# saforem2/l2hmc

Measured on AMD Instinct MI355X. Metric: leapfrog-steps/sec (whole node), 8x8 U(1) batch 2048, 10 LF, higher is better.
Workload: dtype f32; 1 GPU; U(1) 8x8 lattice, beta=2.0, batch 2048 per GPU, 10 LF steps, GenericNet H=512 (BASELINE.json configs[2]); global_batch=2048, num_steps=10, parallelism=chains sharded over 1 GPU(s) (weak scaling), weights replicated

## Files before the change

include/l2hmc_hip.h:

```cpp
#ifndef L2HMC_HIP_H
#define L2HMC_HIP_H

#include <stddef.h>
#include <stdint.h>

#ifdef __cplusplus
extern "C" {
#endif

#define L2HMC_OK 0
#define L2HMC_ERR_ARG 1
#define L2HMC_ERR_HIP 2
#define L2HMC_ERR_WORKSPACE 3

#define L2HMC_ABI_VERSION 1

typedef void* l2hmc_stream_t;

int l2hmc_abi_version(void);
const char* l2hmc_last_error(void);

int l2hmc_u1_action_force(const float* x, int64_t rows, int32_t T, int32_t X, float beta,
                          float* action, float* force, float* avg_plaq, float* top_charge,
                          l2hmc_stream_t stream);
// ... 37 lines not shown
size_t l2hmc_stq_ws_bytes(int64_t rows, int32_t H);

int l2hmc_stq_dense(const l2hmc_dense_net* net, const float* a, const float* b, const float* bmask,
                    float t_cos, float t_sin, int64_t rows, float* S, float* T, float* Q,
                    void* ws, size_t ws_bytes, l2hmc_stream_t stream);

size_t l2hmc_stq_conv3d_ws_bytes(int64_t rows, int32_t H, int32_t T, int32_t X, int32_t F);
int l2hmc_stq_conv3d(const l2hmc_conv3d_front* front, const l2hmc_dense_net* net, int32_t T, int32_t X,
                     const float* a, const float* b, const float* bmask, float t_cos, float t_sin,
                     int64_t rows, float* S, float* Tr, float* Q, void* ws, size_t ws_bytes,
                     l2hmc_stream_t stream);

int l2hmc_lf_update_v(const float* v, const float* grad, const float* S, const float* T,
                      const float* Q, float eps, int32_t dir, int64_t rows, int32_t D,
                      float* v_out, float* logdet, l2hmc_stream_t stream);
int l2hmc_lf_update_x(const float* x, const float* v, const float* keep, const float* S,
                      const float* T, const float* Q, float eps, int32_t dir, int64_t rows,
                      int32_t D, float* x_out, float* logdet, l2hmc_stream_t stream);

int l2hmc_accept_prob(const float* h_old, const float* h_new, const float* sumlogdet, int64_t n,
                      float* p, l2hmc_stream_t stream);

int l2hmc_mix_accept(const float* x, const float* xf, const float* vf, const float* pf,
                     const float* xb, const float* vb, const float* pb, const float* coin,
                     const float* u, int32_t strict, int64_t B, int32_t D, float* x_prop,
                     float* v_prop, float* p, float* x_out, l2hmc_stream_t stream);

#define L2HMC_PLAN_LAYERED 1
#define L2HMC_PLAN_CONV3D 2
#define L2HMC_PLAN_SELECTED_ONLY 4
#define L2HMC_PLAN_RECOMPUTE 8
#define L2HMC_PLAN_TILES16_ONLY 16
#define L2HMC_PLAN_ALL_COLUMNS 32
typedef struct l2hmc_gauge_plan {
  int32_t T, X;
  int32_t num_steps;
  int32_t hmc;
  float eps;
  int32_t flags;
  const float* masks;
  l2hmc_dense_net xnet;
  l2hmc_dense_net vnet;
  l2hmc_conv3d_front xfront;
  l2hmc_conv3d_front vfront;
  const void* heads;
} l2hmc_gauge_plan;

size_t l2hmc_gauge_pack_heads_bytes(const l2hmc_gauge_plan* plan);
int l2hmc_gauge_pack_heads(const l2hmc_gauge_plan* plan, void* heads, l2hmc_stream_t stream);

size_t l2hmc_gauge_ws_bytes(const l2hmc_gauge_plan* plan, int64_t rows);

int l2hmc_gauge_plan_fused(const l2hmc_gauge_plan* plan);

int l2hmc_gauge_step_plan(int64_t rows_all, int32_t cus, int64_t* rows_out, int32_t* rows_per_wg_out);

int l2hmc_gauge_leapfrog(const l2hmc_gauge_plan* plan, float beta, int32_t step, float* x, float* v,
                         const int32_t* dir, int64_t rows, float* logdet, void* ws, size_t ws_bytes,
                         l2hmc_stream_t stream);

int l2hmc_gauge_trajectory(const l2hmc_gauge_plan* plan, float beta, const float* x0, const float* v0,
                           const int32_t* dir, int64_t rows, float* x_out, float* v_out,
                           float* sumlogdet, float* p_accept, void* ws, size_t ws_bytes,
                           l2hmc_stream_t stream);

size_t l2hmc_gauge_transition_ws_bytes(const l2hmc_gauge_plan* plan, int64_t B, int32_t both_directions);
// ... 160 lines not shown
```

l2hmc_amd/_lib.py:

```python
import ctypes as C
import os
import re

import torch

_HERE = os.path.dirname(os.path.abspath(__file__))
LIB_PATH = os.environ.get("L2HMC_LIB_PATH") or os.path.join(_HERE, "libl2hmc_hip.so")
HEADER_PATH = os.path.join(os.path.dirname(_HERE), "include", "l2hmc_hip.h")

c_float_p = C.c_void_p
MAX_MIX, MAX_SMALL_DIM, MAX_SMALL_NODES = 8, 8, 64
PLAN_LAYERED, PLAN_CONV3D, PLAN_SELECTED_ONLY, PLAN_RECOMPUTE, PLAN_TILES16_ONLY, PLAN_ALL_COLUMNS = 1, 2, 4, 8, 16, 32
GRAD_BUCKET_REST = 6
BUCKET_FN = C.CFUNCTYPE(None, C.c_void_p, C.c_int32)


class DenseNet(C.Structure):
    _fields_ = [("D", C.c_int32), ("H", C.c_int32), ("Ka", C.c_int32), ("Kb", C.c_int32),
                ("w1_t", c_float_p), ("wt", c_float_p), ("b1", c_float_p), ("wh_t", c_float_p),
                ("bh", c_float_p), ("whd_t", c_float_p), ("bhd", c_float_p),
                ("coeff_s", c_float_p), ("coeff_q", c_float_p),
                ("q_tanh", C.c_int32), ("reserved", C.c_int32), ("packed", c_float_p)]


class DenseGrads(C.Structure):
    _fields_ = [(n, c_float_p) for n in ("w1_t", "wt", "b1", "wh_t", "bh", "whd_t", "bhd", "coeff_s", "coeff_q")]


class Conv3DGrads(C.Structure):
    _fields_ = [(n, c_float_p) for n in ("w1_a", "b1_a", "w2_a", "b2_a", "w1_b", "b1_b", "w2_b", "b2_b")]


class Conv3DFront(C.Structure):
    _fields_ = [("F", C.c_int32), ("reserved", C.c_int32),
                ("w1_a", c_float_p), ("b1_a", c_float_p), ("w2_a", c_float_p), ("b2_a", c_float_p),
                ("w1_b", c_float_p), ("b1_b", c_float_p), ("w2_b", c_float_p), ("b2_b", c_float_p)]


class GaugePlan(C.Structure):
    _fields_ = [("T", C.c_int32), ("X", C.c_int32), ("num_steps", C.c_int32), ("hmc", C.c_int32),
                ("eps", C.c_float), ("flags", C.c_int32), ("masks", c_float_p),
                ("xnet", DenseNet), ("vnet", DenseNet), ("xfront", Conv3DFront), ("vfront", Conv3DFront),
                ("heads", C.c_void_p)]


# ... 184 lines not shown
```

l2hmc_amd/csrc/fused_args.h:

```cpp
#pragma once
#include "stq_dense.h"

namespace l2hmc {

struct FusedArgs {
  int T, X, num_steps, step_begin, step_end;
  float eps, beta;
  const float* masks;
  l2hmc_dense_net xnet, vnet;
  l2hmc_conv3d_front xfront, vfront;
  const float* x0; const float* v0;
  const int* dir;
  int64_t x_mod;
  int64_t dir_split;
  int64_t rows;
  float* x_out; float* v_out;
  float* logdet;
  int logdet_accumulate;
  float* p_accept;
  unsigned long long* stamps;
  int stagger;
  FusedTape tx, tv;
  float* step_x_next;
  float* step_xprop; float* step_vprop; float* step_xout;
  int64_t step_B;
  int64_t step_Bl, step_chain0;
  int step_sums_acc;
  unsigned long long step_seed, step_draw;
  int step_both;
  float* step_px; float* step_act; float* step_plq; float* step_chg; float* step_dq;
  float* step_sums;
  float* step_part;
  int step_split;
  float* step_hand;
  int* step_ticket;
  const int* heads_meta;
  const float* heads_img;
};

size_t fused4_pack_floats(const l2hmc_dense_net* n);
int launch_fused4_pack(const l2hmc_dense_net* n, float* image4, hipStream_t stream);
int fused4_rows_per_wg(int64_t rows, int cus);
int launch_fused4(const FusedArgs& a, int rows_per_wg, hipStream_t stream);

int fused32_supported(const l2hmc_dense_net* n);
int launch_fused32(const FusedArgs& a, hipStream_t stream);

}
```

l2hmc_amd/csrc/fused_traj.hip:

```cpp
#include "fused_step.h"
#include <atomic>
#include <stdlib.h>

namespace l2hmc {

template <int D, int H, int KA = D, bool CONV = false>
struct FusedCfg {
  static constexpr int IMGW = CONV ? 2 * kFWaves : kFWaves;
  static constexpr int WAVES = 2 * kFWaves;
  static constexpr int RW = WAVES / IMGW;
  static constexpr int THREADS = 64 * WAVES;
  static constexpr int TPC = CONV ? THREADS / kFM : 16;
  static constexpr int SX = D + 8;
  static constexpr int SA = KA + 8;
  static constexpr int SH = H + 8;
  static constexpr int NT1 = H / (16 * WAVES);
  static constexpr int NTH = D / (16 * WAVES);
  static constexpr int NTI1 = H / (16 * IMGW);
  static constexpr int NTIH = D / (16 * IMGW);
  static_assert(NT1 >= 1 && NT1 <= 8 && NTH >= 1, "every wave needs at least one tile per layer");
  static_assert(RW == 1 || NTH == 1, "a shared heads section is walked with one tile per head and wave");
  static constexpr int KC1 = 2 * KA / 16;
  static constexpr int KC2 = H / 16;
  static constexpr size_t P1 = (size_t)2 * KA * H;
  static constexpr size_t P2 = (size_t)H * H;
  static constexpr size_t PH = (size_t)3 * D * H;
  static constexpr int NC = 4 * H + 5 * D;
  static constexpr int CF = 8, CL = 8;
  static constexpr int CW = 18 * CF + CF + 8 * CF * CF + 2 * CF;
  static constexpr int CXIN = (CL + 2) * (CL + 2) * 2;
  static constexpr int CP1 = (CL / 2 + 1) * (CL / 2 + 1) * CF;
  static constexpr int CONV_FLOATS = CONV ? 2 * kFM * SA + 4 * CW + kFM * (CXIN + CP1) : 0;
  static constexpr int ACT_FLOATS = CONV ? 0 : kFM * SX + D + 4;
  static constexpr int LDS_FLOATS = 3 * kFM * SX + 2 * kFM * SH + 2 * NC + kFM * (D / 2 + 4)  +
                                    2 * D  + WAVES * kFM  + (RW > 1 ? IMGW * 64 : 0)  + kFM  +
                                    8 * kFM  + CONV_FLOATS + ACT_FLOATS;
};

__global__ void pack_fused_kernel(l2hmc_dense_net n, float* __restrict__ out, int waves) {
  const int kFWaves = waves;
  const int D = n.D, H = n.H, K1 = n.Ka + n.Kb;
  const size_t P1 = (size_t)K1 * H, P2 = (size_t)H * H, PH = (size_t)3 * D * H;
  const int NT1 = H / (16 * kFWaves), NTH = D / (16 * kFWaves);
  for (size_t i = (size_t)blockIdx.x * blockDim.x + threadIdx.x; i < P1 + P2 + PH;
       i += (size_t)gridDim.x * blockDim.x) {
    const int j = (int)(i & 3), lane = (int)((i >> 2) & 63);
    size_t rest;
    float val;
    if (i < P1 + P2) {
      const bool first = i < P1;
      const int K = first ? K1 : H;
      rest = (first ? i : i - P1) >> 8;
      const int t = (int)(rest % NT1);
      rest /= NT1;
      const int KC = K / 16;
      const int kc = (int)(rest % KC), w = (int)(rest / KC);
      const int col = (w * NT1 + t) * 16 + (lane & 15);
      const int k = kc * 16 + (lane >> 4) * 4 + j;
      val = first ? n.w1_t[(size_t)col * K1 + k] : n.wh_t[(size_t)col * H + k];
    } else {
      rest = (i - P1 - P2) >> 8;
      const int t = (int)(rest % NTH);
      rest /= NTH;
      const int hd = (int)(rest % 3);
      rest /= 3;
      const int KC = H / 16;
      const int kc = (int)(rest % KC), w = (int)(rest / KC);
      const int col = w * (D / kFWaves) + t * 16 + (lane & 15);
      const int k = kc * 16 + (lane >> 4) * 4 + j;
      val = n.whd_t[((size_t)hd * D + col) * H + k];
    }
    out[i] = val;
  }
}

__global__ __launch_bounds__(256) void pack_heads_kernel(l2hmc_dense_net n, const float* __restrict__ masks, int N,
                                                         int* __restrict__ meta, float* __restrict__ img) {
  constexpr int DMAX = 128;
  __shared__ int cols[DMAX / 2];
  __shared__ int ok;
  const int D = n.D, H = n.H, DA = D / 2;
  const float* row = masks + (size_t)(blockIdx.y >> 1) * D;
  const float sense = (float)(blockIdx.y & 1);
  if (threadIdx.x == 0) {
    int cnt = 0, bin = D <= DMAX;
    for (int c = 0; c < D && bin; ++c) {
      const float v = row[c];
      if (!(v == 0.f || v == 1.f)) bin = 0;
      else if (v == sense) {
        if (cnt < DA) cols[cnt] = c;
        ++cnt;
      }
    }
    ok = bin && cnt == DA;
  }
  __syncthreads();
  if (blockIdx.x == 0) {
    if (threadIdx.x == 0) meta[blockIdx.y] = ok;
    for (int i = threadIdx.x; i < DA; i += blockDim.x) meta[2 * N + (size_t)blockIdx.y * DA + i] = ok ? cols[i] : -1;
  }
  if (!ok) return;
  const size_t per = (size_t)3 * DA * H;
  float* out = img + (size_t)blockIdx.y * per;
  const int KC = H / 16;
  for (size_t i = (size_t)blockIdx.x * blockDim.x + threadIdx.x; i < per; i += (size_t)gridDim.x * blockDim.x) {
    const int j = (int)(i & 3), lane = (int)((i >> 2) & 63);
    size_t rest = i >> 8;
    const int hd = (int)(rest % 3);
    rest /= 3;
    const int kc = (int)(rest % KC), w = (int)(rest / KC);
    const int col = cols[w * 16 + (lane & 15)];
    const int k = kc * 16 + (lane >> 4) * 4 + j;
    out[i] = n.whd_t[((size_t)hd * D + col) * H + k];
  }
}

#ifdef L2HMC_STAMPS
#define FT_NOW()                                                                              \
  ({                                                                                          \
    unsigned long long t_;                                                                    \
    __builtin_amdgcn_sched_barrier(0);                                                        \
    asm volatile("s_memtime %0\n\ts_waitcnt lgkmcnt(0)" : "=s"(t_)::"memory");                \
    __builtin_amdgcn_sched_barrier(0);                                                        \
    t_;                                                                                       \
  })
#define FT_ADD(slot, t0) ft[slot] += FT_NOW() - (t0)
#else
#define FT_NOW() 0ull
#define FT_ADD(slot, t0) do {} while (0)
#endif


#ifdef L2HMC_STAMPS
int g_fused_stagger = 0;
extern "C" void l2hmc_debug_set_stagger(int cycles) { g_fused_stagger = cycles; }
#endif

template <int D, int H, int KA, bool CONV, bool TAPE = false>
__global__ __launch_bounds__((FusedCfg<D, H, KA, CONV>::THREADS)) void gauge_traj_fused_kernel(FusedArgs p) {
  using Cfg = FusedCfg<D, H, KA, CONV>;
  constexpr int kFWaves = Cfg::WAVES, kFThreads = Cfg::THREADS, kTPC = Cfg::TPC;
  constexpr int SX = Cfg::SX, SH = Cfg::SH, SA = Cfg::SA, NT1 = Cfg::NT1, NTH = Cfg::NTH;
  constexpr int RW = Cfg::RW, IMGW = Cfg::IMGW, NTI1 = Cfg::NTI1, NTIH = Cfg::NTIH;
  constexpr int TSH = RW > 1 ? NTIH : 1;
  constexpr int sites = D / 2;
  constexpr int SP = sites + 4;
  extern __shared__ __attribute__((aligned(16))) float lds[];
  float* xs = lds;
  float* vs = xs + kFM * SX;
  float* gs = vs + kFM * SX;
  float* h1 = gs + kFM * SX;
  float* h2 = h1 + kFM * SH;
  float* cx = h2 + kFM * SH;
  float* cv = cx + Cfg::NC;
  float* sp = cv + Cfg::NC;
  float* skm = sp + kFM * SP;
  float* ldw = skm + 2 * D;
  float* ldx = ldw + IMGW * kFM;
  int* sdir = reinterpret_cast<int*>(ldw + kFWaves * kFM + (RW > 1 ? IMGW * 64 : 0));
  float* stp = reinterpret_cast<float*>(sdir + kFM);
  float* fa = stp + 8 * kFM;
  float* fb = fa + kFM * SA;
  float* cwl = fb + kFM * SA;
  float* cxin = cwl + 4 * Cfg::CW;
  float* cp1 = cxin + kFM * Cfg::CXIN;
  float* stg = stp + 8 * kFM + Cfg::CONV_FLOATS;
  int* scol = reinterpret_cast<int*>(stg + kFM * SX);
  int* sel = scol + D;

  [[maybe_unused]] unsigned long long ft[10] = {0, 0, 0, 0, 0, 0, 0, 0, 0, 0};
  [[maybe_unused]] const unsigned long long ft_start = FT_NOW();
#ifdef L2HMC_STAMPS
  unsigned long long rt0;
  asm volatile("s_memrealtime %0\n\ts_waitcnt lgkmcnt(0)" : "=s"(rt0)::"memory");
#endif
  const int tid = threadIdx.x;
  const int lane = tid & 63, wave = tid >> 6;
  const int q = lane >> 4, r = lane & 15;
  const int64_t row0 = (int64_t)blockIdx.x * kFM;
  const int nrow = (int)min((int64_t)kFM, p.rows - row0);
  const float eps = p.eps;

#ifdef L2HMC_STAMPS
  if (p.stagger > 0) {
    const long long delay = (long long)((blockIdx.x >> 3) & 31) * p.stagger;
    const long long t0 = (long long)__builtin_amdgcn_s_memtime();
    while ((long long)__builtin_amdgcn_s_memtime() - t0 < delay) __builtin_amdgcn_s_sleep(16);
  }
#endif
  const bool SPLIT = !CONV && !TAPE && p.step_B > 0 && p.step_both && p.step_split;
  const StepWg wg = step_workgroup<kFM>(p, stp, SPLIT);
  const bool STEPM = wg.stepm;
  const int sdw = wg.sdw;
  float* spx = wg.spx;
  stage_chains<kFM, kFThreads, D, SX>(p, wg, xs, vs, sdir);
  load_consts<kFThreads, D, H>(p.xnet, cx, tid);
  load_consts<kFThreads, D, H>(p.vnet, cv, tid);
  if constexpr (CONV) {
    constexpr int F = Cfg::CF, F2 = 2 * Cfg::CF;
    auto load_filters = [&](const float* w1, const float* b1, const float* w2, const float* b2, float* dst) {
      for (int i = tid; i < 18 * F; i += kFThreads) dst[i] = w1[i];
      for (int i = tid; i < F; i += kFThreads) dst[18 * F + i] = b1[i];
      for (int i = tid; i < 4 * F * F2; i += kFThreads) {
        const int g = i % F2, c = (i / F2) % F, tap = i / (F2 * F);
        dst[19 * F + i] = w2[((size_t)(tap * 2) * F + c) * F2 + g];
      }
      for (int i = tid; i < F2; i += kFThreads) dst[19 * F + 4 * F * F2 + i] = b2[i];
    };
    load_filters(p.xfront.w1_a, p.xfront.b1_a, p.xfront.w2_a, p.xfront.b2_a, cwl + 0 * Cfg::CW);
    load_filters(p.xfront.w1_b, p.xfront.b1_b, p.xfront.w2_b, p.xfront.b2_b, cwl + 1 * Cfg::CW);
    load_filters(p.vfront.w1_a, p.vfront.b1_a, p.vfront.w2_a, p.vfront.b2_a, cwl + 2 * Cfg::CW);
    load_filters(p.vfront.w1_b, p.vfront.b1_b, p.vfront.w2_b, p.vfront.b2_b, cwl + 3 * Cfg::CW);
    for (int i = tid; i < kFM * (Cfg::CXIN + Cfg::CP1); i += kFThreads) cxin[i] = 0.f;
  }
  if (tid < IMGW * kFM) ldw[tid] = 0.f;
  __syncthreads();

  const int dirl = sdir[r];

  const ChainLanes cl = chain_lanes<kFM, kTPC, 1>(p, tid);
  float act0[1], kin0[1];
  force_pass<kFM, kTPC, 1, D, SX, SP>(cl, xs, sp, gs, act0);
  kinetic_pass<kFM, kTPC, 1, D, SX>(cl, vs, kin0);

  [[maybe_unused]] auto conv_features = [&](const float* src, const float* cw, float* dst) {
    constexpr int F = Cfg::CF, F2 = 2 * Cfg::CF, L = Cfg::CL, LP = L + 2, L2 = L / 2, L2P = L2 + 1, L4 = L / 4;
    const float* w1 = cw;
    const float* b1 = cw + 18 * F;
    const float* w2 = b1 + F;
    const float* b2 = w2 + 4 * F * F2;
    for (int i = tid; i < kFM * D; i += kFThreads) {
      const int c = i / D, e = i - c * D;
      const int site = e >> 1, mu = e & 1, ii = site / L, jj = site - ii * L;
      cxin[c * Cfg::CXIN + ((ii + 1) * LP + jj + 1) * 2 + mu] = src[c * SX + e];
    }
    __syncthreads();
    {
      using f32x2 = __attribute__((ext_vector_type(2))) float;
      constexpr int FP = F / 2;
      static_assert(kFThreads % FP == 0 && F % 2 == 0, "filter pairs must stay with their threads");
      const int fp = tid % FP;
      f32x2 k0[9], k1[9];
#pragma unroll
      for (int t = 0; t < 9; ++t) {
        k0[t] = *reinterpret_cast<const f32x2*>(w1 + (t * 2 + 0) * F + 2 * fp);
        k1[t] = *reinterpret_cast<const f32x2*>(w1 + (t * 2 + 1) * F + 2 * fp);
      }
      const f32x2 bias = *reinterpret_cast<const f32x2*>(b1 + 2 * fp);
// ... 93 lines not shown
        const float* stsrc = mode == 1 ? vs : xs;
        for (int i = tid; i < kFM * (D / 4); i += kFThreads) {
          const int rr = i / (D / 4), c4 = (i - rr * (D / 4)) * 4;
          if (rr < nrow) {
            float* dst = tp.in + (tcr0 + rr) * (2 * D);
            tape_store(dst + c4, *reinterpret_cast<const f32x4*>(in1 + rr * SX + c4));
            tape_store(dst + D + c4, *reinterpret_cast<const f32x4*>(gs + rr * SX + c4));
            tape_store(tp.st + (tcr0 + rr) * D + c4, *reinterpret_cast<const f32x4*>(stsrc + rr * SX + c4));
          }
        }
      }
    }
    [[maybe_unused]] auto tape_rows = [&](float* dst, const float* src) {
      for (int i = tid; i < kFM * (H / 4); i += kFThreads) {
        const int rr = i / (H / 4), c4 = (i - rr * (H / 4)) * 4;
        if (rr < nrow)
          tape_store(dst + (tcr0 + rr) * H + c4, *reinterpret_cast<const f32x4*>(src + rr * SH + c4));
      }
    };
    const int wv = __builtin_amdgcn_readfirstlane(wave);
    const int wimg = wv / RW, wsub = wv - wimg * RW;
    const float* wp1 = pk + (size_t)wimg * Cfg::KC1 * NTI1 * 256;
    const float* wp2 = pk + Cfg::P1 + (size_t)wimg * Cfg::KC2 * NTI1 * 256;
    const float* wph = pk + Cfg::P1 + Cfg::P2 + (size_t)wimg * Cfg::KC2 * 3 * NTIH * 256;
    const int to1 = wsub * NT1, toh = wsub * NTH;
    int asense = 0;
    bool actv = false;
    const float* wpa = nullptr;
    if (ACTOK && SPLIT && mode == 2 && p.heads_img) {
      asense = sdw ^ sub;
      actv = __builtin_amdgcn_readfirstlane(sel[asense]) != 0;
      wpa = p.heads_img + ((size_t)(arow * 2 + asense) * 4 + (wv & 3)) * Cfg::KC2 * 3 * 256;
    }
    [[maybe_unused]] float ld_k[4] = {0.f, 0.f, 0.f, 0.f}, ld_s[4] = {0.f, 0.f, 0.f, 0.f};
#ifndef L2HMC_DP1
#define L2HMC_DP1 3
#define L2HMC_DP2 3
#define L2HMC_DPH 4
#endif
    constexpr int DP1 = L2HMC_DP1, DP2 = L2HMC_DP2, DPH = L2HMC_DPH;
    BRing<NT1, DP2> R2;
    BRing<3 * NTH, DPH> R3;
    {
      constexpr int KH = Cfg::KC1 / 2;
      f32x4 acc[NT1];
      [[maybe_unused]] unsigned long long t0 = FT_NOW();
      const float* src1 = in1;
      const float* src2 = gs;
      int s1 = SX;
      if constexpr (CONV) {
        const float* cwn = cwl + (is_vnet ? 2 : 0) * Cfg::CW;
        [[maybe_unused]] const unsigned long long tc0 = FT_NOW();
        if (l1 == 0 || l1 == 1 || l1 == 3) conv_features(in1, cwn, fa);
        if (l1 != 2) conv_features(gs, cwn + Cfg::CW, fb);
        FT_ADD(8, tc0);
        src1 = fa;
        src2 = fb;
        s1 = SA;
        if constexpr (TAPE) {
          for (int i = tid; i < kFM * (2 * KA / 4); i += kFThreads) {
            const int rr = i / (2 * KA / 4), c4 = (i - rr * (2 * KA / 4)) * 4;
            if (rr < nrow)
              tape_store(tp.feat + (tcr0 + rr) * (2 * KA) + c4,
                         *reinterpret_cast<const f32x4*>((c4 < KA ? fa + rr * SA + c4 : fb + rr * SA + (c4 - KA))));
          }
        }
      }
      if (l1 == 2) {
#pragma unroll
        for (int t = 0; t < NT1; ++t) acc[t] = keep_v[t];
      } else {
        BRing<NT1, DP1> RA, RB;
        const float* wpb = wp1 + (size_t)KH * NTI1 * 256;
        ring_prime<NT1, DP1, NTI1>(RB, wpb, false, 0, to1);
        if (l1 == 4) {
#pragma unroll
          for (int t = 0; t < NT1; ++t) acc[t] = keep_x[t];
        } else {
          ring_prime<NT1, DP1, NTI1>(RA, wp1, false, 0, to1);
#pragma unroll
          for (int t = 0; t < NT1; ++t) acc[t] = f32x4{0.f, 0.f, 0.f, 0.f};
          const float* a1 = src1 + r * s1 + q * 4;
          stream_layer<NT1, KH, DP1, NTI1>(
              RA, wp1, [&](int kc) { return *reinterpret_cast<const f32x4*>(a1 + kc * 16); }, acc, false, to1);
          if (l1 == 3) {
#pragma unroll
            for (int t = 0; t < NT1; ++t) keep_x[t] = acc[t];
          }
        }
        const float* a2 = src2 + r * s1 + q * 4;
        stream_layer<NT1, KH, DP1, NTI1>(
            RB, wpb, [&](int kc) { return *reinterpret_cast<const f32x4*>(a2 + kc * 16); }, acc, false, to1);
        if (l1 == 1) {
#pragma unroll
          for (int t = 0; t < NT1; ++t) keep_v[t] = acc[t];
        }
      }
      ring_prime<NT1, DP2, NTI1>(R2, wp2, zig, Cfg::KC2, to1);
      FT_ADD(0, t0);
      t0 = FT_NOW();
      [[maybe_unused]] unsigned gmask = 0;
#pragma unroll
      for (int t = 0; t < NT1; ++t) {
        const int c0 = (wave * NT1 + t) * 16 + q * 4;
        const f32x4 b = *reinterpret_cast<const f32x4*>(cn + c0);
        const f32x4 w0 = *reinterpret_cast<const f32x4*>(cn + H + c0);
        const f32x4 w1 = *reinterpret_cast<const f32x4*>(cn + 2 * H + c0);
        f32x4 hv;
#pragma unroll
        for (int e = 0; e < 4; ++e) {
          hv[e] = fmaxf(acc[t][e] + b[e] + (tcr * w0[e] + tsr * w1[e]), 0.f);
          if constexpr (TAPE) gmask |= (hv[e] > 0.f ? 1u : 0u) << (t * 4 + e);
        }
        *reinterpret_cast<f32x4*>(h1 + r * SH + c0) = hv;
      }
      if constexpr (TAPE) {
        const size_t word = ((size_t)(callidx * 2 + 0) * gridDim.x + blockIdx.x) * (64 * IMGW) + wimg * 64 + lane;
        if constexpr (RW == 1) tp.gate[word] = gmask;
        else reinterpret_cast<unsigned short*>(tp.gate)[word * 2 + wsub] = (unsigned short)gmask;
      }
      FT_ADD(3, t0);
    }
    {
      [[maybe_unused]] const unsigned long long tb = FT_NOW();
      __syncthreads();
// ... 54 lines not shown
      } else {
        stream_layer<3 * NTH, Cfg::KC2, DPH, 3 * NTIH, TSH>(
            R3, wph, [&](int kc) { return *reinterpret_cast<const f32x4*>(a + kc * 16); }, acc, zig, toh);
      }
      FT_ADD(2, t0);
      t0 = FT_NOW();
      float ld = 0.f;
      const float* bhd = cn + 4 * H;
      const float* es = bhd + 3 * D;
      const float* eq = es + D;
      const int d = dirl;
      if (ACTOK && actv) {
        const int* al = scol + asense * (D / 2);
        const int* il = scol + (asense ^ 1) * (D / 2);
        if (wv < 4) {
#pragma unroll
          for (int e = 0; e < 4; ++e) {
            const int c = al[wv * 16 + q * 4 + e];
            const int idx = r * SX + c;
            const float S = fast_tanh(acc[0][e] + bhd[c]) * es[c];
            const float Tt = acc[1][e] + bhd[D + c];
            const float qq = acc[2][e] + bhd[2 * D + c];
            const float Q = (net.q_tanh ? fast_tanh(qq) : qq) * eq[c];
            const float mf = skm[c], mb = skm[D + c];
            const float keep = sub == 0 ? (d ? 1.f - mb : mf) : (d ? mb : 1.f - mf);
            const float x = xs[idx], v = vs[idx];
            const float s = (d ? -eps : eps) * S;
            const float drift = eps * (fast_exp(eps * Q) * v + Tt);
            const float es_ = fast_exp(s);
            const float upd = d ? es_ * (x - drift) : x * es_ + drift;
            const float xn = keep * x + (1.f - keep) * upd;
            xs[idx] = xn;
            stg[idx] = (1.f - keep) * s;
            if (prep_next_mask) gs[idx] = (1.f - keep) * xn;
          }
        } else {
#pragma unroll
          for (int e = 0; e < 4; ++e) {
            const int c = il[(wv - 4) * 16 + q * 4 + e];
            const int idx = r * SX + c;
            stg[idx] = 0.f;
            if (prep_next_mask) {
              const float mf = skm[c], mb = skm[D + c];
              const float keep = sub == 0 ? (d ? 1.f - mb : mf) : (d ? mb : 1.f - mf);
              gs[idx] = (1.f - keep) * xs[idx];
            }
          }
        }
      } else {
#pragma unroll
      for (int t = 0; t < NTH; ++t) {
        const int c0 = wave * (D / kFWaves) + t * 16 + q * 4;
        const f32x4 b_s = *reinterpret_cast<const f32x4*>(bhd + c0);
        const f32x4 b_t = *reinterpret_cast<const f32x4*>(bhd + D + c0);
        const f32x4 b_q = *reinterpret_cast<const f32x4*>(bhd + 2 * D + c0);
        const f32x4 e_s = *reinterpret_cast<const f32x4*>(es + c0);
        const f32x4 e_q = *reinterpret_cast<const f32x4*>(eq + c0);
        const f32x4 mf = *reinterpret_cast<const f32x4*>(skm + c0);
        const f32x4 mb = *reinterpret_cast<const f32x4*>(skm + D + c0);
        const int idx = r * SX + c0;
        f32x4 S, Tt, Q;
#pragma unroll
        for (int e = 0; e < 4; ++e) {
          S[e] = fast_tanh(acc[0 * NTH + t][e] + b_s[e]) * e_s[e];
          Tt[e] = acc[1 * NTH + t][e] + b_t[e];
          const float qq = acc[2 * NTH + t][e] + b_q[e];
          Q[e] = (net.q_tanh ? fast_tanh(qq) : qq) * e_q[e];
        }
        if constexpr (TAPE) {
          if (r < nrow) {
            const size_t plane = (size_t)p.rows * D;
            float* o = tp.stq + (size_t)callidx * 3 * plane + ((size_t)row0 + r) * D + c0;
            tape_store(o, S);
            tape_store(o + plane, Tt);
            tape_store(o + 2 * plane, Q);
          }
        }
        if (mode == 1) {
          const f32x4 g = *reinterpret_cast<const f32x4*>(gs + idx);
          const f32x4 v = *reinterpret_cast<const f32x4*>(vs + idx);
          f32x4 vn;
#pragma unroll
          for (int e = 0; e < 4; ++e) {
            const float s = (d ? -0.5f : 0.5f) * eps * S[e];
            const float kick = 0.5f * eps * (fast_exp(eps * Q[e]) * g[e] - Tt[e]);
            const float es_ = fast_exp(s);
            vn[e] = d ? es_ * (v[e] + kick) : v[e] * es_ - kick;
            ld += s;
            if constexpr (RW > 1) { ld_k[e] = 1.f; ld_s[e] = s; }
          }
          *reinterpret_cast<f32x4*>(vs + idx) = vn;
          if (prep_next_mask) {
            const f32x4 x = *reinterpret_cast<const f32x4*>(xs + idx);
            f32x4 kx;
#pragma unroll
            for (int e = 0; e < 4; ++e) kx[e] = (d ? 1.f - mb[e] : mf[e]) * x[e];
            *reinterpret_cast<f32x4*>(gs + idx) = kx;
          }
        } else {
          const f32x4 x = *reinterpret_cast<const f32x4*>(xs + idx);
          const f32x4 v = *reinterpret_cast<const f32x4*>(vs + idx);
          f32x4 xn, kx;
#pragma unroll
          for (int e = 0; e < 4; ++e) {
            const float keep = sub == 0 ? (d ? 1.f - mb[e] : mf[e]) : (d ? mb[e] : 1.f - mf[e]);
            const float s = (d ? -eps : eps) * S[e];
            const float drift = eps * (fast_exp(eps * Q[e]) * v[e] + Tt[e]);
            const float es_ = fast_exp(s);
            const float upd = d ? es_ * (x[e] - drift) : x[e] * es_ + drift;
            xn[e] = keep * x[e] + (1.f - keep) * upd;
            ld += (1.f - keep) * s;
            if constexpr (RW > 1) { ld_k[e] = 1.f - keep; ld_s[e] = s; }
            kx[e] = (1.f - keep) * xn[e];
          }
          *reinterpret_cast<f32x4*>(xs + idx) = xn;
          if (prep_next_mask) *reinterpret_cast<f32x4*>(gs + idx) = kx;
        }
      }
      if constexpr (RW == 1) {
        ld += __shfl_xor(ld, 16, 64);
        ld += __shfl_xor(ld, 32, 64);
        if (q == 0) ldw[wave * kFM + r] += ld;
      } else {
        if (wsub == 0) ldx[wimg * 64 + lane] = ld;
      }
      }
      FT_ADD(5, t0);
    }
    {
      [[maybe_unused]] const unsigned long long tb = FT_NOW();
// ... 7 lines not shown
        for (int h = 0; h < 2; ++h)
#pragma unroll
          for (int e = 0; e < 4; ++e) ld += stg[r * SX + (2 * wimg + h) * 16 + q * 4 + e];
        ld += __shfl_xor(ld, 16, 64);
        ld += __shfl_xor(ld, 32, 64);
        if (q == 0) ldw[wimg * kFM + r] += ld;
      }
    } else if constexpr (RW > 1) {
      if (wsub == 1) {
        float ld = ldx[wimg * 64 + lane];
#pragma unroll
        for (int e = 0; e < 4; ++e) ld += ld_k[e] * ld_s[e];
        ld += __shfl_xor(ld, 16, 64);
        ld += __shfl_xor(ld, 32, 64);
        if (q == 0) ldw[wimg * kFM + r] += ld;
      }
    }
  };

  const float two_pi = 6.28318530717958647692f;
  for (int step = p.step_begin; step < p.step_end; ++step) {
    const int sf = step, sb = p.num_steps - 1 - step;
    const float af = two_pi * (float)sf / (float)p.num_steps, ab = two_pi * (float)sb / (float)p.num_steps;
    const float tcf = cosf(af), tsf = sinf(af), tcb = cosf(ab), tsb = sinf(ab);
    const float tcr = dirl ? tcb : tcf, tsr = dirl ? tsb : tsf;
    for (int i = tid; i < D; i += kFThreads) {
      skm[i] = p.masks[(size_t)sf * D + i];
      skm[D + i] = p.masks[(size_t)sb * D + i];
    }
    if (ACTOK && SPLIT && p.heads_meta) {
      arow = sdw ? sb : sf;
      for (int i = tid; i < D; i += kFThreads) scol[i] = p.heads_meta[2 * p.num_steps + arow * D + i];
      if (tid < 2) sel[tid] = p.heads_meta[arow * 2 + tid];
    }
    __syncthreads();
#pragma nounroll
    for (int call = 0; call < 4; ++call) {
      const bool is_v = call == 0 || call == 3;
      if (call == 3) {
        [[maybe_unused]] const unsigned long long tf = FT_NOW();
        float unused[1];
        force_pass<kFM, kTPC, 1, D, SX, SP>(cl, xs, sp, gs, unused);
        FT_ADD(7, tf);
      }
      const int l1 = call == 0 ? (keep_v_valid ? 2 : 0) : call == 1 ? 3 : call == 2 ? 4 : 1;
      net_update(is_v ? p.vnet : p.xnet, is_v ? cv : cx, is_v ? xs : vs, is_v ? 1 : 2, call == 2 ? 1 : 0,
                 call < 2, l1, is_v, tcr, tsr, 2 * step + (call == 0 || call == 1 ? 0 : 1));
    }
    keep_v_valid = true;
  }

  float act1[1], kin1[1];
  force_pass<kFM, kTPC, 1, D, SX, SP>(cl, xs, sp, gs, act1);
  kinetic_pass<kFM, kTPC, 1, D, SX>(cl, vs, kin1);
  if (STEPM) {
    step_accept_probs<kFM, 1, IMGW>(cl, ldw, act0, act1, kin0, kin1, spx);
    __syncthreads();
    const float* xfr = xs;
    const float* xbr = xs + (kFM / 2) * SX;
    const float* vfr = vs;
    const float* vbr = vs + (kFM / 2) * SX;
    const float* pfr = spx;
    const float* pbr = spx + kFM / 2;
    if (SPLIT) {
      constexpr int HW = 2 * kFM * D + kFM;
      float* mine = p.step_hand + (size_t)blockIdx.x * HW;
// ... 35 lines not shown
      if (sdw == 0) {
        xbr = ox; vbr = ov; pbr = op;
      } else {
        xfr = ox; vfr = ov; pfr = op;
        xbr = xs; vbr = vs; pbr = spx;
      }
    }
    float* gin = gs;
    float* gout = h1;
    step_mix_accept<kFThreads, D, SX>(p, wg, xfr, xbr, vfr, vbr, pfr, pbr, gin, gout);
    step_observables<kFM, kTPC, 1, D, SX>(p, wg, cl, gin, gout);
    const int ngrp = SPLIT ? 2 : 1;
    const int64_t slot0 = SPLIT ? (int64_t)(blockIdx.x >> 1) * 2 : (int64_t)blockIdx.x;
    const int nfin = SPLIT ? (int)(gridDim.x >> 1) : (int)gridDim.x;
    const int npart = SPLIT ? (int)((p.step_Bl + kFM / 2 - 1) / (kFM / 2)) : (int)gridDim.x;
    step_sums<kFThreads, kFThreads>(p, wg, ngrp, slot0, npart, nfin, vs);
    step_write_next<kFThreads, D, SX>(p, wg, gout);
    return;
  }
  traj_logdet_accept<kFM, 1, IMGW>(p, wg, cl, ldw, act0, act1, kin0, kin1);
#ifdef L2HMC_STAMPS
  if (p.stamps && tid == 0) {
    unsigned long long rt1;
    asm volatile("s_memrealtime %0\n\ts_waitcnt lgkmcnt(0)" : "=s"(rt1)::"memory");
    ft[9] = FT_NOW() - ft_start;
    for (int i = 0; i < 10; ++i) p.stamps[blockIdx.x * 12 + i] = ft[i];
    p.stamps[blockIdx.x * 12 + 10] = rt0;
    p.stamps[blockIdx.x * 12 + 11] = rt1;
  }
#endif
  traj_write_back<kFM, kFThreads, D, SX>(p, wg, xs, vs);
}

static size_t heads_meta_bytes(int N, int D) { return align_up(sizeof(int) * ((size_t)2 * N + (size_t)N * D), 256); }
static int fused_generic_net(const l2hmc_dense_net* n) {
  return n->D == 128 && n->H == 512 && n->Ka == 128 && n->Kb == 128;
}
static int fused_conv_net(const l2hmc_dense_net* n) {
  return n->D == 128 && n->H == 256 && n->Ka == 64 && n->Kb == 64;
}
int fused_net_supported(const l2hmc_dense_net* n) { return fused_generic_net(n) || fused_conv_net(n); }

static bool subtile_enabled(const l2hmc_gauge_plan* p) { return !(p->flags & L2HMC_PLAN_TILES16_ONLY); }
static int device_cu_count() {
  static std::atomic<int> cached[16];
  int dev = 0;
  if (hipGetDevice(&dev) != hipSuccess || dev < 0 || dev >= 16) return 256;
  int n = cached[dev].load(std::memory_order_relaxed);
  if (n <= 0) {
    if (hipDeviceGetAttribute(&n, hipDeviceAttributeMultiprocessorCount, dev) != hipSuccess || n <= 0) n = 256;
    cached[dev].store(n, std::memory_order_relaxed);
  }
  return n;
}
int fused_plan_supported(const l2hmc_gauge_plan* p) {
  if (p->hmc || !p->xnet.packed || !p->vnet.packed || 2 * p->T * p->X != 128 || (p->X & (p->X - 1)) != 0) return 0;
  if (p->flags & L2HMC_PLAN_CONV3D)
    return fused_conv_net(&p->xnet) && fused_conv_net(&p->vnet) && p->T == 8 && p->X == 8 && p->xfront.F == 8 &&
           p->vfront.F == 8;
  return fused_generic_net(&p->xnet) && fused_generic_net(&p->vnet);
}

int launch_fused_trajectory(const l2hmc_gauge_plan* p, float beta, int step_begin, int step_end,
                            const float* x0, const float* v0, const int* dir, int64_t rows, float* x_out,
                            float* v_out, float* logdet, int logdet_accumulate, float* p_accept,
                            hipStream_t stream, int64_t x_mod, int64_t dir_split, const FusedTape* tape_x,
                            const FusedTape* tape_v) {
// ... 135 lines not shown
    step_once.done();
  }
  L2HMC_REQUIRE(x_in && (x_next || x_out) && B > 0 && (!step_sums || part) && hand, "fused step: bad arguments");
  const int ndir = both ? 2 : 1;
  StepPart parts[3];
  const int nparts = plan_step_parts(B * ndir, !conv && subtile_enabled(p), device_cu_count(), parts);
  auto part_of = [&](int64_t c0, int64_t nb, int rpw, int accumulate) {
    const int cpw = both ? rpw / 2 : rpw;
    const int64_t D = 2 * (int64_t)p->T * p->X;
    FusedArgs a{};
    a.T = p->T; a.X = p->X; a.num_steps = p->num_steps; a.step_begin = 0; a.step_end = p->num_steps;
    a.eps = p->eps; a.beta = beta; a.masks = p->masks; a.xnet = p->xnet; a.vnet = p->vnet;
    a.xfront = p->xfront; a.vfront = p->vfront;
    a.x0 = x_in + c0 * D; a.rows = ceil_div(nb, cpw) * rpw;
    a.step_x_next = x_next ? x_next + c0 * D : nullptr;
    a.step_xprop = x_prop ? x_prop + c0 * D : nullptr;
    a.step_vprop = v_prop ? v_prop + c0 * D : nullptr;
    a.step_xout = x_out ? x_out + c0 * D : nullptr;
    a.step_B = B; a.step_Bl = nb; a.step_chain0 = c0; a.step_sums_acc = accumulate;
    a.step_seed = seed; a.step_draw = draw; a.step_both = both;
    a.step_px = px ? px + c0 : nullptr; a.step_act = actions ? actions + c0 : nullptr;
    a.step_plq = plaqs ? plaqs + c0 : nullptr; a.step_chg = charges ? charges + c0 : nullptr;
    a.step_dq = dq ? dq + c0 : nullptr;
    a.step_sums = step_sums; a.step_part = part;
#ifdef L2HMC_STAMPS
    a.stamps = g_stamp_cls == 5 ? g_stamp_buf : nullptr;
    a.stagger = g_fused_stagger;
#endif
    return a;
  };
  const bool split = !conv && both;
  const int* hmeta = nullptr;
  const float* himg = nullptr;
  if (split && p->heads && !(p->flags & L2HMC_PLAN_ALL_COLUMNS)) {
    hmeta = reinterpret_cast<const int*>(p->heads);
    himg = reinterpret_cast<const float*>(reinterpret_cast<const char*>(p->heads) +
                                          heads_meta_bytes(p->num_steps, 2 * p->T * p->X));
  }
  auto launch16 = [&](FusedArgs a) {
    if (split) {
      const int64_t pairs = ceil_div(a.step_Bl, (int64_t)kFM);
      a.rows = 2 * pairs * kFM;
      a.step_split = 1;
      a.step_ticket = static_cast<int*>(hand);
      a.step_hand = reinterpret_cast<float*>(static_cast<char*>(hand) + hand_ticket_bytes(pairs));
      a.heads_meta = hmeta;
      a.heads_img = himg;
      if (hipMemsetAsync(a.step_ticket, 0, sizeof(int) * (size_t)pairs, stream) != hipSuccess) {
        set_error("fused step: cannot clear the hand-off tickets");
        return L2HMC_ERR_HIP;
      }
    }
    const unsigned nwg = (unsigned)(a.rows / kFM);
    prof_before(kProfFused, stream);
    if (conv)
      hipLaunchKernelGGL((gauge_traj_fused_kernel<128, 256, 64, true>), dim3(nwg), dim3(CfgC::THREADS), lds, stream, a);
    else
      hipLaunchKernelGGL((gauge_traj_fused_kernel<128, 512, 128, false>), dim3(nwg), dim3(CfgG::THREADS), lds, stream, a);
    prof_after(kProfFused, stream);
    L2HMC_CHECK_LAUNCH("gauge_traj_fused (step)");
    return L2HMC_OK;
  };
  int64_t c0 = 0;
  for (int i = 0; i < nparts; ++i) {
    const int64_t nb = parts[i].rows / ndir;
    const FusedArgs a = part_of(c0, nb, parts[i].rpw, i > 0);
    if (int e = parts[i].rpw == 32 ? launch_fused32(a, stream)
                : parts[i].rpw == kFM ? launch16(a) : launch_fused4(a, parts[i].rpw, stream))
      return e;
    c0 += nb;
  }
  return L2HMC_OK;
}

}

using namespace l2hmc;

extern "C" size_t l2hmc_gauge_pack_heads_bytes(const l2hmc_gauge_plan* plan) {
  if (!plan || plan->hmc || plan->num_steps <= 0 || (plan->flags & L2HMC_PLAN_CONV3D) || 2 * plan->T * plan->X != 128 ||
      !fused_generic_net(&plan->xnet))
    return 0;
  const int D = 128, H = plan->xnet.H;
  return heads_meta_bytes(plan->num_steps, D) + sizeof(float) * (size_t)2 * plan->num_steps * 3 * (D / 2) * H;
}

extern "C" int l2hmc_gauge_pack_heads(const l2hmc_gauge_plan* plan, void* buf, l2hmc_stream_t stream) {
  L2HMC_REQUIRE(plan != nullptr && buf != nullptr, "gauge_pack_heads: NULL pointer");
  L2HMC_REQUIRE(l2hmc_gauge_pack_heads_bytes(plan) > 0, "gauge_pack_heads: the plan has no active-column heads "
                "(GenericNet D = 128, H = 512 on an 8x8-site lattice, hmc = 0)");
  L2HMC_REQUIRE(plan->masks && plan->xnet.whd_t, "gauge_pack_heads: NULL masks or heads weights");
  const int N = plan->num_steps, D = 128;
  int* meta = static_cast<int*>(buf);
  float* img = reinterpret_cast<float*>(static_cast<char*>(buf) + heads_meta_bytes(N, D));
  hipLaunchKernelGGL(pack_heads_kernel, dim3(32, (unsigned)(2 * N)), dim3(256), 0, (hipStream_t)stream, plan->xnet,
                     plan->masks, N, meta, img);
  L2HMC_CHECK_LAUNCH("gauge_pack_heads");
  return L2HMC_OK;
}

extern "C" size_t l2hmc_dense_pack_bytes(const l2hmc_dense_net* net) {
  if (!net || !fused_net_supported(net)) return 0;
  return sizeof(float) * ((size_t)(net->Ka + net->Kb) * net->H + (size_t)net->H * net->H + (size_t)3 * net->D * net->H +
                          fused4_pack_floats(net));
}

extern "C" int l2hmc_dense_pack(const l2hmc_dense_net* net, float* packed, l2hmc_stream_t stream) {
  L2HMC_REQUIRE(net != nullptr && packed != nullptr, "dense_pack: NULL pointer");
  L2HMC_REQUIRE(fused_net_supported(net), "dense_pack: shape (D=%d, H=%d, Ka=%d, Kb=%d) has no fused kernel",
                net->D, net->H, net->Ka, net->Kb);
  L2HMC_REQUIRE(net->w1_t && net->wh_t && net->whd_t, "dense_pack: NULL weight pointer");
  const int waves = fused_conv_net(net) ? FusedCfg<128, 256, 64, true>::IMGW : FusedCfg<128, 512, 128, false>::IMGW;
  hipLaunchKernelGGL(pack_fused_kernel, dim3(1024), dim3(256), 0, (hipStream_t)stream, *net, packed, waves);
  L2HMC_CHECK_LAUNCH("dense_pack");
  if (fused4_pack_floats(net))
    return launch_fused4_pack(net, packed + (size_t)(net->Ka + net->Kb) * net->H + (size_t)net->H * net->H +
                                        (size_t)3 * net->D * net->H, (hipStream_t)stream);
  return L2HMC_OK;
}
```

l2hmc_amd/gauge_dynamics.py:

```python
import ctypes as C

import numpy as np
import numpy.random as npr
import torch

from . import _lib
from . import autograd as _autograd
from .network import ConvNet3D, GenericNet


class GaugeDynamics:

    def __init__(self, lattice, potential_fn, **kwargs):
        self.name = 'GaugeDynamics'
        self.lattice = lattice
        self.potential = potential_fn
        self.batch_size = self.lattice.samples.shape[0]
        self.x_dim = self.lattice.num_links
        self.hmc, self.network_arch, self.num_steps = False, 'generic', 5
        self.eps_trainable, self.data_format = True, 'channels_last'
        self.both_directions = True
        self.fused = True
        self.check_numerics = False
        self.recompute = False
        self.tiles16_only = False
        self.all_columns = False
        for key, val in kwargs.items():
            if key != 'eps':
                setattr(self, key, val)
        self._device = kwargs.get('device') or torch.device("cuda", torch.cuda.current_device())
        if getattr(potential_fn, "u1_lattice", None) is None:
            raise NotImplementedError(
                "the fused trajectory integrates the 2D U(1) action; pass lattice.get_energy_function()")
        self.eps = torch.tensor(float(kwargs.get('eps', 0.4)), dtype=torch.float32)
        self._construct_time()
        self._construct_masks_while()
        if self.hmc:
            self.position_fn = lambda inp: [torch.zeros_like(inp[0]) for _ in range(3)]
            self.momentum_fn = lambda inp: [torch.zeros_like(inp[0]) for _ in range(3)]
        elif self.network_arch == 'generic':
            self._build_generic_nets()
        elif self.network_arch == 'conv3D':
            self._build_conv_nets_3D()
        elif self.network_arch == 'conv2D':
            raise NotImplementedError(
                "network_arch='conv2D' is out of scope (SURVEY.md section 2: not named by any benchmark "
                "config, and its 4-D outputs break the reference's own reduce_sum(axis=1))")
        else:
            raise AttributeError("`self._network_arch` must be one of `'conv3D', 'conv2D', 'generic'.`")
        self._ws = _lib.Workspace()
        self._seed = int(kwargs.get('seed', 42))
        self._draws = 0

    def _build_generic_nets(self):
        kwargs = {'x_dim': self.x_dim, 'links_shape': self.lattice.links.shape,
                  'num_hidden': int(4 * self.x_dim), 'name_scope': 'position', 'factor': 2.}
        self.position_fn = GenericNet(model_name='XNet', device=self._device, **kwargs)
        kwargs['factor'] = 1.
        kwargs['name_scope'] = 'momentum'
# ... 28 lines not shown
            idx = npr.permutation(np.arange(self.x_dim))[:self.x_dim // 2]
            mask = np.zeros((self.x_dim,))
            mask[idx] = 1
            mask_per_step.append(mask)
        self.set_masks(np.stack(mask_per_step))

    def set_masks(self, masks):
        masks = np.asarray(masks, dtype=np.float32)
        if masks.shape != (self.num_steps, self.x_dim):
            raise ValueError(f"masks: expected {(self.num_steps, self.x_dim)}, got {masks.shape}")
        self.mask = _lib.as_dev(masks, self._device)

    @property
    def variables(self):
        v = [self.eps]
        if not self.hmc:
            v += self.position_fn.variables + self.momentum_fn.variables
        return v

    @property
    def trainable_variables(self):
        v = [self.eps] if self.eps_trainable else []
        if not self.hmc:
            v += self.position_fn.trainable_variables + self.momentum_fn.trainable_variables
        return v

    def _plan(self):
        p = _lib.GaugePlan(T=self.lattice.time_size, X=self.lattice.space_size, num_steps=self.num_steps,
                           hmc=int(bool(self.hmc)), eps=float(self.eps.detach()),
                           flags=(0 if self.fused else _lib.PLAN_LAYERED)
                           | (0 if self.both_directions else _lib.PLAN_SELECTED_ONLY)
                           | (_lib.PLAN_RECOMPUTE if self.recompute else 0)
                           | (_lib.PLAN_TILES16_ONLY if self.tiles16_only else 0)
                           | (_lib.PLAN_ALL_COLUMNS if self.all_columns else 0),
                           masks=_lib.dev_ptr(self.mask, name="mask"))
        if not self.hmc:
            p.xnet = self.position_fn.pack()
            p.vnet = self.momentum_fn.pack()
            if self.network_arch == 'conv3D':
                p.flags |= _lib.PLAN_CONV3D
                p.xfront = self.position_fn.pack_front()
                p.vfront = self.momentum_fn.pack_front()
            elif self.fused:
                p.heads = self._heads_image(p)
        return p

    def _heads_image(self, plan):
        L = _lib.lib()
        nbytes = L.l2hmc_gauge_pack_heads_bytes(C.byref(plan))
        if not nbytes:
            return None
        key = (plan.xnet.whd_t, getattr(self.position_fn, "_pack_serial", 0))
        h = getattr(self, "_heads", None)
        if h is None or h[0] is not self.mask or h[1] != key or h[2].numel() * 4 < nbytes:
            buf = torch.empty(nbytes // 4, dtype=torch.float32, device=self._device)
            _lib.check(L.l2hmc_gauge_pack_heads(C.byref(plan), buf.data_ptr(), _lib.stream_ptr(self._device)))
            self._heads = h = (self.mask, key, buf)
        return h[2].data_ptr()

    def _x(self, a):
        a = _lib.as_dev(a, self._device)
        return a.reshape(a.shape[0], -1)

    def _normal(self, shape):
        out = torch.empty(shape, dtype=torch.float32, device=self._device)
        _lib.check(_lib.lib().l2hmc_fill_normal(out.data_ptr(), out.numel(), self._seed, self._draws,
                                                _lib.stream_ptr(self._device)))
# ... 165 lines not shown
```

Baseline: 15.40 million chain-leapfrog-steps/s.

## Compact masked x-input columns in first layer to halve its K dimension

Packs a per-step compacted copy of the first-layer weights that keeps only the x-input columns not zeroed by the mask, plus a column-position map in the heads metadata. The fused trajectory kernel then streams half the K range for the masked x-input of layer one, writing the masked activations straight into compacted positions. This removes multiply-adds against inputs that are always zero. NaN propagation from the dropped columns is kept through a per-row flag. The cost is extra packed weight memory, extra LDS, and more complex staging logic. The old full-width path stays available behind a new FULL_L1 plan flag.

```diff
diff --git a/include/l2hmc_hip.h b/include/l2hmc_hip.h
--- a/include/l2hmc_hip.h
+++ b/include/l2hmc_hip.h
@@ -93,6 +93,7 @@
 #define L2HMC_PLAN_RECOMPUTE 8
 #define L2HMC_PLAN_TILES16_ONLY 16
 #define L2HMC_PLAN_ALL_COLUMNS 32
+#define L2HMC_PLAN_FULL_L1 64
 typedef struct l2hmc_gauge_plan {
   int32_t T, X;
   int32_t num_steps;
diff --git a/l2hmc_amd/_lib.py b/l2hmc_amd/_lib.py
--- a/l2hmc_amd/_lib.py
+++ b/l2hmc_amd/_lib.py
@@ -11,6 +11,7 @@
 c_float_p = C.c_void_p
 MAX_MIX, MAX_SMALL_DIM, MAX_SMALL_NODES = 8, 8, 64
 PLAN_LAYERED, PLAN_CONV3D, PLAN_SELECTED_ONLY, PLAN_RECOMPUTE, PLAN_TILES16_ONLY, PLAN_ALL_COLUMNS = 1, 2, 4, 8, 16, 32
+PLAN_FULL_L1 = 64
 GRAD_BUCKET_REST = 6
 BUCKET_FN = C.CFUNCTYPE(None, C.c_void_p, C.c_int32)
 
diff --git a/l2hmc_amd/csrc/fused_args.h b/l2hmc_amd/csrc/fused_args.h
--- a/l2hmc_amd/csrc/fused_args.h
+++ b/l2hmc_amd/csrc/fused_args.h
@@ -36,6 +36,7 @@
   int* step_ticket;
   const int* heads_meta;
   const float* heads_img;
+  const float* l1_img;
 };
 
 size_t fused4_pack_floats(const l2hmc_dense_net* n);
diff --git a/l2hmc_amd/csrc/fused_traj.hip b/l2hmc_amd/csrc/fused_traj.hip
--- a/l2hmc_amd/csrc/fused_traj.hip
+++ b/l2hmc_amd/csrc/fused_traj.hip
@@ -31,7 +31,7 @@
   static constexpr int CXIN = (CL + 2) * (CL + 2) * 2;
   static constexpr int CP1 = (CL / 2 + 1) * (CL / 2 + 1) * CF;
   static constexpr int CONV_FLOATS = CONV ? 2 * kFM * SA + 4 * CW + kFM * (CXIN + CP1) : 0;
-  static constexpr int ACT_FLOATS = CONV ? 0 : kFM * SX + D + 4;
+  static constexpr int ACT_FLOATS = CONV ? 0 : kFM * SX + D + 4 + D + 2 * kFM;
   static constexpr int LDS_FLOATS = 3 * kFM * SX + 2 * kFM * SH + 2 * NC + kFM * (D / 2 + 4)  +
                                     2 * D  + WAVES * kFM  + (RW > 1 ? IMGW * 64 : 0)  + kFM  +
                                     8 * kFM  + CONV_FLOATS + ACT_FLOATS;
@@ -74,12 +74,16 @@
   }
 }
 
+__host__ __device__ inline int kept_compact_k(int n) { return (n & ~15) + 4 * (n & 3) + ((n >> 2) & 3); }
+
 __global__ __launch_bounds__(256) void pack_heads_kernel(l2hmc_dense_net n, const float* __restrict__ masks, int N,
-                                                         int* __restrict__ meta, float* __restrict__ img) {
+                                                         int* __restrict__ meta, float* __restrict__ img,
+                                                         int* __restrict__ cpos, float* __restrict__ img1) {
   constexpr int DMAX = 128;
   __shared__ int cols[DMAX / 2];
+  __shared__ int kcol[DMAX / 2];
   __shared__ int ok;
-  const int D = n.D, H = n.H, DA = D / 2;
+  const int D = n.D, H = n.H, DA = D / 2, K1 = n.Ka + n.Kb;
   const float* row = masks + (size_t)(blockIdx.y >> 1) * D;
   const float sense = (float)(blockIdx.y & 1);
   if (threadIdx.x == 0) {
@@ -93,11 +97,24 @@
       }
     }
     ok = bin && cnt == DA;
+    if (ok) {
+      int nk = 0;
+      for (int w = 0; w < D; ++w) {
+        const int c = (w & ~15) + 4 * (w & 3) + ((w >> 2) & 3);
+        if (row[c] != sense) kcol[kept_compact_k(nk++)] = c;
+      }
+    }
   }
   __syncthreads();
   if (blockIdx.x == 0) {
     if (threadIdx.x == 0) meta[blockIdx.y] = ok;
     for (int i = threadIdx.x; i < DA; i += blockDim.x) meta[2 * N + (size_t)blockIdx.y * DA + i] = ok ? cols[i] : -1;
+    int* cp = cpos + (size_t)(blockIdx.y >> 1) * D;
+    if (ok) {
+      for (int i = threadIdx.x; i < DA; i += blockDim.x) cp[kcol[i]] = i;
+    } else {
+      for (int i = threadIdx.x; i < D; i += blockDim.x) cp[i] = -1;
+    }
   }
   if (!ok) return;
   const size_t per = (size_t)3 * DA * H;
@@ -112,6 +129,19 @@
     const int col = cols[w * 16 + (lane & 15)];
     const int k = kc * 16 + (lane >> 4) * 4 + j;
     out[i] = n.whd_t[((size_t)hd * D + col) * H + k];
+  }
+  const size_t per1 = (size_t)DA * H;
+  float* out1 = img1 + (size_t)blockIdx.y * per1;
+  const int KC1 = DA / 16, NT = H / (16 * 4);
+  for (size_t i = (size_t)blockIdx.x * blockDim.x + threadIdx.x; i < per1; i += (size_t)gridDim.x * blockDim.x) {
+    const int j = (int)(i & 3), lane = (int)((i >> 2) & 63);
+    size_t rest = i >> 8;
+    const int t = (int)(rest % NT);
+    rest /= NT;
+    const int kc = (int)(rest % KC1), w = (int)(rest / KC1);
+    const int col = (w * NT + t) * 16 + (lane & 15);
+    const int k = kc * 16 + (lane >> 4) * 4 + j;
+    out1[i] = n.w1_t[(size_t)col * K1 + n.Ka + kcol[k]];
   }
 }
 
@@ -167,6 +197,8 @@
   float* stg = stp + 8 * kFM + Cfg::CONV_FLOATS;
   int* scol = reinterpret_cast<int*>(stg + kFM * SX);
   int* sel = scol + D;
+  int* scp = sel + 4;
+  float* spz = reinterpret_cast<float*>(scp + D);
 
   [[maybe_unused]] unsigned long long ft[10] = {0, 0, 0, 0, 0, 0, 0, 0, 0, 0};
   [[maybe_unused]] const unsigned long long ft_start = FT_NOW();
@@ -214,6 +246,9 @@
     for (int i = tid; i < kFM * (Cfg::CXIN + Cfg::CP1); i += kFThreads) cxin[i] = 0.f;
   }
   if (tid < IMGW * kFM) ldw[tid] = 0.f;
+  if constexpr (!CONV) {
+    if (tid < 2 * kFM) spz[tid] = 0.f;
+  }
   __syncthreads();
 
   const int dirl = sdir[r];
@@ -373,6 +408,7 @@
       actv = __builtin_amdgcn_readfirstlane(sel[asense]) != 0;
       wpa = p.heads_img + ((size_t)(arow * 2 + asense) * 4 + (wv & 3)) * Cfg::KC2 * 3 * 256;
     }
+    const bool l1c = ACTOK && SPLIT && p.l1_img && p.heads_img && __builtin_amdgcn_readfirstlane(sel[0] & sel[1]) != 0;
     [[maybe_unused]] float ld_k[4] = {0.f, 0.f, 0.f, 0.f}, ld_s[4] = {0.f, 0.f, 0.f, 0.f};
 #ifndef L2HMC_DP1
 #define L2HMC_DP1 3
@@ -412,7 +448,9 @@
         for (int t = 0; t < NT1; ++t) acc[t] = keep_v[t];
       } else {
         BRing<NT1, DP1> RA, RB;
+        const bool cmp = l1c && mode == 2;
         const float* wpb = wp1 + (size_t)KH * NTI1 * 256;
+        if (cmp) wpb = p.l1_img + ((size_t)(arow * 2 + asense) * IMGW + wimg) * (KH / 2) * NTI1 * 256;
         ring_prime<NT1, DP1, NTI1>(RB, wpb, false, 0, to1);
         if (l1 == 4) {
 #pragma unroll
@@ -429,9 +467,30 @@
             for (int t = 0; t < NT1; ++t) keep_x[t] = acc[t];
           }
         }
-        const float* a2 = src2 + r * s1 + q * 4;
-        stream_layer<NT1, KH, DP1, NTI1>(
-            RB, wpb, [&](int kc) { return *reinterpret_cast<const f32x4*>(a2 + kc * 16); }, acc, false, to1);
+        bool x_done = false;
+        if constexpr (ACTOK) {
+          if (cmp) {
+            x_done = true;
+            const float* a2 = (sub == 0 ? stg : gs) + r * SX + q * 4;
+            const bool bad = spz[sub * kFM + r] != 0.f;
+            stream_layer<NT1, KH / 2, DP1, NTI1>(
+                RB, wpb,
+                [&](int kc) {
+                  f32x4 a = *reinterpret_cast<const f32x4*>(a2 + kc * 16);
+                  if (kc == 0) {
+#pragma unroll
+                    for (int e = 0; e < 4; ++e) a[e] = bad ? __builtin_nanf("") : a[e];
+                  }
+                  return a;
+                },
+                acc, false, to1);
+          }
+        }
+        if (!x_done) {
+          const float* a2 = src2 + r * s1 + q * 4;
+          stream_layer<NT1, KH, DP1, NTI1>(
+              RB, wpb, [&](int kc) { return *reinterpret_cast<const f32x4*>(a2 + kc * 16); }, acc, false, to1);
+        }
         if (l1 == 1) {
 #pragma unroll
           for (int t = 0; t < NT1; ++t) keep_v[t] = acc[t];
@@ -552,7 +611,7 @@
             const float xn = keep * x + (1.f - keep) * upd;
             xs[idx] = xn;
             stg[idx] = (1.f - keep) * s;
-            if (prep_next_mask) gs[idx] = (1.f - keep) * xn;
+            if (prep_next_mask) gs[l1c ? r * SX + scp[c] : idx] = (1.f - keep) * xn;
           }
         } else {
 #pragma unroll
@@ -563,9 +622,12 @@
             if (prep_next_mask) {
               const float mf = skm[c], mb = skm[D + c];
               const float keep = sub == 0 ? (d ? 1.f - mb : mf) : (d ? mb : 1.f - mf);
-              gs[idx] = (1.f - keep) * xs[idx];
+              const float kx = (1.f - keep) * xs[idx];
+              if (!l1c) gs[idx] = kx;
+              else if (kx != kx) spz[kFM + r] = kx;
             }
           }
+          if (l1c && wv == 4 && q == 0) spz[sub * kFM + r] = 0.f;
         }
       } else {
 #pragma unroll
@@ -615,7 +677,15 @@
             f32x4 kx;
 #pragma unroll
             for (int e = 0; e < 4; ++e) kx[e] = (d ? 1.f - mb[e] : mf[e]) * x[e];
-            *reinterpret_cast<f32x4*>(gs + idx) = kx;
+            if (l1c) {
+#pragma unroll
+              for (int e = 0; e < 4; ++e) {
+                if ((d ? 1.f - mb[e] : mf[e]) != 0.f) stg[r * SX + scp[c0 + e]] = kx[e];
+                else if (kx[e] != kx[e]) spz[r] = kx[e];
+              }
+            } else {
+              *reinterpret_cast<f32x4*>(gs + idx) = kx;
+            }
           }
         } else {
           const f32x4 x = *reinterpret_cast<const f32x4*>(xs + idx);
@@ -689,6 +759,8 @@
       arow = sdw ? sb : sf;
       for (int i = tid; i < D; i += kFThreads) scol[i] = p.heads_meta[2 * p.num_steps + arow * D + i];
       if (tid < 2) sel[tid] = p.heads_meta[arow * 2 + tid];
+      if (p.l1_img)
+        for (int i = tid; i < D; i += kFThreads) scp[i] = p.heads_meta[2 * p.num_steps + (p.num_steps + arow) * D + i];
     }
     __syncthreads();
 #pragma nounroll
@@ -790,7 +862,9 @@
   traj_write_back<kFM, kFThreads, D, SX>(p, wg, xs, vs);
 }
 
-static size_t heads_meta_bytes(int N, int D) { return align_up(sizeof(int) * ((size_t)2 * N + (size_t)N * D), 256); }
+static size_t heads_meta_bytes(int N, int D) { return align_up(sizeof(int) * ((size_t)2 * N + (size_t)2 * N * D), 256); }
+static size_t heads_sections_bytes(int N, int D, int H) { return sizeof(float) * (size_t)2 * N * 3 * (D / 2) * H; }
+static size_t l1_sections_bytes(int N, int D, int H) { return sizeof(float) * (size_t)2 * N * (D / 2) * H; }
 static int fused_generic_net(const l2hmc_dense_net* n) {
   return n->D == 128 && n->H == 512 && n->Ka == 128 && n->Kb == 128;
 }
@@ -992,10 +1066,14 @@
   const bool split = !conv && both;
   const int* hmeta = nullptr;
   const float* himg = nullptr;
+  const float* l1img = nullptr;
   if (split && p->heads && !(p->flags & L2HMC_PLAN_ALL_COLUMNS)) {
+    const int Dp = 2 * p->T * p->X;
     hmeta = reinterpret_cast<const int*>(p->heads);
-    himg = reinterpret_cast<const float*>(reinterpret_cast<const char*>(p->heads) +
-                                          heads_meta_bytes(p->num_steps, 2 * p->T * p->X));
+    himg = reinterpret_cast<const float*>(reinterpret_cast<const char*>(p->heads) + heads_meta_bytes(p->num_steps, Dp));
+    if (!(p->flags & L2HMC_PLAN_FULL_L1))
+      l1img = reinterpret_cast<const float*>(reinterpret_cast<const char*>(himg) +
+                                             heads_sections_bytes(p->num_steps, Dp, p->xnet.H));
   }
   auto launch16 = [&](FusedArgs a) {
     if (split) {
@@ -1006,6 +1084,7 @@
       a.step_hand = reinterpret_cast<float*>(static_cast<char*>(hand) + hand_ticket_bytes(pairs));
       a.heads_meta = hmeta;
       a.heads_img = himg;
+      a.l1_img = l1img;
       if (hipMemsetAsync(a.step_ticket, 0, sizeof(int) * (size_t)pairs, stream) != hipSuccess) {
         set_error("fused step: cannot clear the hand-off tickets");
         return L2HMC_ERR_HIP;
@@ -1042,19 +1121,21 @@
       !fused_generic_net(&plan->xnet))
     return 0;
   const int D = 128, H = plan->xnet.H;
-  return heads_meta_bytes(plan->num_steps, D) + sizeof(float) * (size_t)2 * plan->num_steps * 3 * (D / 2) * H;
+  return heads_meta_bytes(plan->num_steps, D) + heads_sections_bytes(plan->num_steps, D, H) +
+         l1_sections_bytes(plan->num_steps, D, H);
 }
 
 extern "C" int l2hmc_gauge_pack_heads(const l2hmc_gauge_plan* plan, void* buf, l2hmc_stream_t stream) {
   L2HMC_REQUIRE(plan != nullptr && buf != nullptr, "gauge_pack_heads: NULL pointer");
   L2HMC_REQUIRE(l2hmc_gauge_pack_heads_bytes(plan) > 0, "gauge_pack_heads: the plan has no active-column heads "
                 "(GenericNet D = 128, H = 512 on an 8x8-site lattice, hmc = 0)");
-  L2HMC_REQUIRE(plan->masks && plan->xnet.whd_t, "gauge_pack_heads: NULL masks or heads weights");
+  L2HMC_REQUIRE(plan->masks && plan->xnet.whd_t && plan->xnet.w1_t, "gauge_pack_heads: NULL masks or weights");
   const int N = plan->num_steps, D = 128;
   int* meta = static_cast<int*>(buf);
   float* img = reinterpret_cast<float*>(static_cast<char*>(buf) + heads_meta_bytes(N, D));
+  float* img1 = reinterpret_cast<float*>(reinterpret_cast<char*>(img) + heads_sections_bytes(N, D, plan->xnet.H));
   hipLaunchKernelGGL(pack_heads_kernel, dim3(32, (unsigned)(2 * N)), dim3(256), 0, (hipStream_t)stream, plan->xnet,
-                     plan->masks, N, meta, img);
+                     plan->masks, N, meta, img, meta + 2 * N + N * D, img1);
   L2HMC_CHECK_LAUNCH("gauge_pack_heads");
   return L2HMC_OK;
 }
diff --git a/l2hmc_amd/gauge_dynamics.py b/l2hmc_amd/gauge_dynamics.py
--- a/l2hmc_amd/gauge_dynamics.py
+++ b/l2hmc_amd/gauge_dynamics.py
@@ -25,6 +25,7 @@
         self.recompute = False
         self.tiles16_only = False
         self.all_columns = False
+        self.full_l1 = False
         for key, val in kwargs.items():
             if key != 'eps':
                 setattr(self, key, val)
@@ -119,7 +120,8 @@
                            | (0 if self.both_directions else _lib.PLAN_SELECTED_ONLY)
                            | (_lib.PLAN_RECOMPUTE if self.recompute else 0)
                            | (_lib.PLAN_TILES16_ONLY if self.tiles16_only else 0)
-                           | (_lib.PLAN_ALL_COLUMNS if self.all_columns else 0),
+                           | (_lib.PLAN_ALL_COLUMNS if self.all_columns else 0)
+                           | (_lib.PLAN_FULL_L1 if self.full_l1 else 0),
                            masks=_lib.dev_ptr(self.mask, name="mask"))
         if not self.hmc:
             p.xnet = self.position_fn.pack()
```

Measured after the change: 15.65 million chain-leapfrog-steps/s (median of 6 runs). 1.02x the previous value.
